# SciSharp/Gym.NET

Measured on AMD Instinct MI355X. Metric: env-steps/sec, higher is better.
Workload: dtype f32

## Files before the change

### gym.net_amd/csrc/lanes.hpp

```cpp
#pragma once
#include <hip/hip_runtime.h>
#include <stdint.h>

namespace gymnet {

template <class T, int N> struct VecOf { typedef T type __attribute__((ext_vector_type(N))); };
typedef float f32x4 __attribute__((ext_vector_type(4)));
typedef int32_t i32x4 __attribute__((ext_vector_type(4)));

template <class T, int VEC>
constexpr int piece_of() { return (int)(16 / sizeof(T)) < VEC ? (int)(16 / sizeof(T)) : VEC; }

template <class T, int VEC, bool NT, bool GUARD>
__device__ __forceinline__ void load_row(const T *__restrict__ p, int64_t i0, int64_t n, T (&v)[VEC]) {
    if constexpr (VEC > 1 && sizeof(T) > 1) {
        if (!GUARD || i0 + VEC <= n) {
            constexpr int P = piece_of<T, VEC>();
            static_assert(VEC % P == 0, "VEC must be a whole number of 16-byte pieces");
            typedef typename VecOf<T, P>::type V;
#pragma unroll
            for (int q = 0; q < VEC / P; ++q) {
                V t;
                if constexpr (NT) t = __builtin_nontemporal_load(reinterpret_cast<const V *>(p + i0 + q * P));
                else t = *reinterpret_cast<const V *>(p + i0 + q * P);
#pragma unroll
                for (int j = 0; j < P; ++j) v[q * P + j] = t[j];
            }
            return;
        }
    }
#pragma unroll
    for (int j = 0; j < VEC; ++j) {
        if (!GUARD || i0 + j < n) { if constexpr (NT) v[j] = __builtin_nontemporal_load(p + i0 + j); else v[j] = p[i0 + j]; }
        else v[j] = T(0);
    }
}

template <class T, int VEC, bool NT, bool GUARD>
__device__ __forceinline__ void store_row(T *__restrict__ p, int64_t i0, int64_t n, const T (&v)[VEC]) {
    if constexpr (VEC > 1 && sizeof(T) > 1) {
        if (!GUARD || i0 + VEC <= n) {
            constexpr int P = piece_of<T, VEC>();
            static_assert(P == 2 || P == 4, "16-byte pieces of 4- or 8-byte elements");
            typedef typename VecOf<T, P>::type V;
#pragma unroll
            for (int q = 0; q < VEC / P; ++q) {
                V t;
                if constexpr (P == 4) t = V{v[q * P], v[q * P + 1], v[q * P + 2], v[q * P + 3]};
                else t = V{v[q * P], v[q * P + 1]};
#ifdef GYMNET_PROBE_STORE_SC1
                if constexpr (NT && sizeof(T) == 4 && P == 4) {
                    asm volatile("global_store_dwordx4 %0, %1, off sc1" :: "v"(p + i0 + q * P), "v"(t) : "memory");
                    continue;
                }
#endif
                if constexpr (NT) __builtin_nontemporal_store(t, reinterpret_cast<V *>(p + i0 + q * P));
                else *reinterpret_cast<V *>(p + i0 + q * P) = t;
            }
            return;
        }
    }
#pragma unroll
    for (int j = 0; j < VEC; ++j)
        if (!GUARD || i0 + j < n) { if constexpr (NT) __builtin_nontemporal_store(v[j], p + i0 + j); else p[i0 + j] = v[j]; }
}

template <int VEC, bool NT, bool GUARD>
__device__ __forceinline__ void store_u8(uint8_t *__restrict__ p, int64_t i0, int64_t n, const uint8_t (&v)[VEC]) {
    if constexpr (VEC == 2) {
        if (!GUARD || i0 + 2 <= n) {
            const uint16_t w = (uint16_t)((uint16_t)v[0] | ((uint16_t)v[1] << 8));
            if constexpr (NT) __builtin_nontemporal_store(w, reinterpret_cast<uint16_t *>(p + i0));
            else *reinterpret_cast<uint16_t *>(p + i0) = w;
            return;
        }
    }
    if constexpr (VEC == 4) {
        if (!GUARD || i0 + 4 <= n) {
            const uint32_t w = (uint32_t)v[0] | ((uint32_t)v[1] << 8) | ((uint32_t)v[2] << 16) | ((uint32_t)v[3] << 24);
            if constexpr (NT) __builtin_nontemporal_store(w, reinterpret_cast<uint32_t *>(p + i0));
            else *reinterpret_cast<uint32_t *>(p + i0) = w;
            return;
        }
    }
#pragma unroll
    for (int j = 0; j < VEC; ++j)
        if (!GUARD || i0 + j < n) { if constexpr (NT) __builtin_nontemporal_store(v[j], p + i0 + j); else p[i0 + j] = v[j]; }
}

template <int VEC, bool NT, bool GUARD>
__device__ __forceinline__ void load_f32(const float *__restrict__ p, int64_t i0, int64_t n, float (&v)[VEC]) { load_row<float, VEC, NT, GUARD>(p, i0, n, v); }
template <int VEC, bool NT, bool GUARD>
__device__ __forceinline__ void store_f32(float *__restrict__ p, int64_t i0, int64_t n, const float (&v)[VEC]) { store_row<float, VEC, NT, GUARD>(p, i0, n, v); }
template <int VEC, bool NT, bool GUARD>
__device__ __forceinline__ void load_i32(const int32_t *__restrict__ p, int64_t i0, int64_t n, int32_t (&v)[VEC]) { load_row<int32_t, VEC, NT, GUARD>(p, i0, n, v); }
template <int VEC, bool NT, bool GUARD>
__device__ __forceinline__ void store_i32(int32_t *__restrict__ p, int64_t i0, int64_t n, const int32_t (&v)[VEC]) { store_row<int32_t, VEC, NT, GUARD>(p, i0, n, v); }

__device__ __forceinline__ uint32_t lane_id() {
    return __builtin_amdgcn_mbcnt_hi(~0u, __builtin_amdgcn_mbcnt_lo(~0u, 0u));
}

}
```

### gym.net_amd/csrc/step_kernels.hpp

```cpp
#pragma once
#include "kernels.hpp"

#include <cstdio>
#include <type_traits>

#include "lanes.hpp"
#include "philox.hpp"

namespace gymnet {

__device__ __forceinline__ float abs_real(float x) { return fabsf(x); }
__device__ __forceinline__ double abs_real(double x) { return __builtin_fabs(x); }

template <class Env, bool UNIFORM_KEY = false>
__device__ __forceinline__ void draw_reset(typename Env::Real (&s)[Env::S], uint64_t key, uint64_t lane, uint64_t tick) {
    if constexpr (Env::RESET_TAKES_KEY) Env::reset(s, key, lane, tick);
    else Env::reset(s, lane_words<UNIFORM_KEY>(key, lane, tick));
}

template <class Env>
__device__ __forceinline__ constexpr bool state_row_own(int k) {
    if constexpr (Env::OBS_ALIASES_STATE) return true; else return Env::OBS_ROW_OF_STATE[k] < 0;
}
template <class Env>
__device__ __forceinline__ const typename Env::Real *state_row_src(const typename Env::Real *state, int64_t state_stride,
                                                                    const typename Env::Real *obs_in, int64_t obs_stride, int k) {
    if constexpr (Env::OBS_ALIASES_STATE) return state + k * state_stride;
    else return Env::OBS_ROW_OF_STATE[k] < 0 ? state + k * state_stride : obs_in + Env::OBS_ROW_OF_STATE[k] * obs_stride;
}

__device__ __forceinline__ uint32_t wave_shard() {
    return (uint32_t)((((int64_t)blockIdx.x * blockDim.x + threadIdx.x) >> 6) & (kShards - 1));
}

template <int VEC, class Args>
__device__ __forceinline__ void count_after_done(const Args &a, const bool (&after)[VEC]) {
    uint32_t total = 0;
#pragma unroll
    for (int j = 0; j < VEC; ++j) total += (uint32_t)__popcll(__ballot(after[j]));
    if (total && lane_id() == (uint32_t)(__ffsll((unsigned long long)__ballot(1)) - 1))
        atomicAdd(&a.after_done[wave_shard() * kAfterStride], (unsigned long long)total);
}

template <class Env, bool AUTORESET, bool SMALL_ANGLE = false>
__device__ __forceinline__ void advance_sublane(typename Env::Real (&sj)[Env::S], typename Env::Action act, int32_t &sbd, float &rw,
                                                bool &dn, bool &after, bool in_range, typename Env::Real (&oj)[Env::O]) {
    if constexpr (Env::HAS_SMALL_ANGLE_PATH) Env::template step<SMALL_ANGLE, AUTORESET>(sj, act, rw, dn);
    else if constexpr (Env::OBS_ALIASES_STATE) Env::step(sj, act, rw, dn);
    else Env::step_observe(sj, act, rw, dn, oj);
    if constexpr (!AUTORESET && Env::HAS_SBD) {
        if (dn) {
            if (sbd == -1) { sbd = 0; }
            else { after = in_range; sbd += 1; rw = 0.0f; }
        }
    }
}

template <class Env, int VEC>
__device__ __forceinline__ bool wave_angles_small(const typename Env::Real (&s)[Env::S][VEC]) {
    if constexpr (!Env::HAS_SMALL_ANGLE_PATH) return false;
    else {
        bool small = true;
#pragma unroll
        for (int j = 0; j < VEC; ++j) small = small && (abs_real(s[Env::ANGLE_ROW][j]) <= Env::SMALL_ANGLE_BOUND);
        return __ballot(!small) == 0;
    }
}

template <class Env, int VEC, bool AUTORESET, bool GUARD, bool PACK = true>
__device__ __forceinline__ void advance_all(typename Env::Real (&s)[Env::S][VEC], typename Env::Action (&act)[VEC], int32_t (&sbd)[VEC],
                                            float (&rw)[VEC], bool (&dn)[VEC], bool (&after)[VEC], typename Env::Real (&o)[Env::O][VEC],
                                            int64_t i0, int64_t n) {
    constexpr int S = Env::S, O = Env::O;
    using Real = typename Env::Real;
#ifndef GYMNET_PROBE_NO_PACK
    constexpr bool kPack = true;
#else
    constexpr bool kPack = false;
#endif
    if constexpr (Env::PACKED2 && VEC == 2 && kPack && PACK) {
        Env::step_observe_x2(s, act, rw, dn, o);
    } else {
        auto all_sublanes = [&](auto small_tag) {
#pragma unroll
            for (int j = 0; j < VEC; ++j) {
// ... 85 lines not shown
    constexpr int S = Env::S;
    using Real = typename Env::Real;
    static_assert(Env::OBS_ALIASES_STATE, "the compacted reset hands back the state only");
    const uint32_t lane = lane_id();
    uint32_t rank[VEC];
    uint32_t total = 0;
#pragma unroll
    for (int j = 0; j < VEC; ++j) {
        const uint64_t m = __ballot((pending >> j) & 1u);
        rank[j] = total + __builtin_amdgcn_mbcnt_hi((uint32_t)(m >> 32), __builtin_amdgcn_mbcnt_lo((uint32_t)m, 0u));
        total += (uint32_t)__popcll(m);
    }
    if (total == 0) return;
    const int64_t wave_i0 = i0 - (int64_t)lane * VEC;
    constexpr bool SPLIT = has_split_reset<Env>();
    const uint32_t active = (uint32_t)__popcll(__ballot(1));
    const uint32_t A = SPLIT ? active >> 1 : active;
    if constexpr (SPLIT) {
        if (A == 0) {
            Real o_unused[Env::O][VEC];
            reset_pending<Env, VEC, LANE_SEEDS>(pending, s, o_unused, a, i0, n, tick);
            return;
        }
    }
    for (uint32_t base = 0; base < total; base += A) {
#pragma unroll
        for (int j = 0; j < VEC; ++j)
            if (((pending >> j) & 1u) && rank[j] - base < A) sc->slot[rank[j] - base] = lane * VEC + (uint32_t)j;
        wave_lds_fence();
        if constexpr (SPLIT) {
            const uint32_t r = lane >> 1, call = lane & 1u;
            const bool draws = r < A && r < total - base;
            PhiloxWords w{};
            if (kResetFullExec || draws) {
                const uint32_t sl = sc->slot[draws ? r : 0u];
                const int64_t gl = wave_i0 + (int64_t)sl;
                uint64_t key = a.seed;
                if constexpr (LANE_SEEDS) {
                    if (a.lane_seed && gl < n) key = a.lane_seed[gl];
                }
                w = lane_words(Env::reset_call_key(key, call), a.lane_offset + (uint64_t)gl, tick);
            }
            const PhiloxWords other = neighbour_words(w);
            if ((kResetFullExec || draws) && call == 0) {
                Real sj[S];
                Env::reset_from_words(sj, w, other);
#pragma unroll
                for (int k = 0; k < S; ++k) sc->draw[r][k] = sj[k];
            }
        } else if (kResetFullExec || lane < total - base) {
            const uint32_t sl = sc->slot[lane < total - base ? lane : 0u];
            const int64_t gl = wave_i0 + (int64_t)sl;
            Real sj[S];
            bool drawn = false;
            if constexpr (LANE_SEEDS) {
                if (a.lane_seed) {
                    draw_reset<Env, false>(sj, gl < n ? a.lane_seed[gl] : a.seed, a.lane_offset + (uint64_t)gl, tick);
                    drawn = true;
                }
            }
            if (!drawn) draw_reset<Env, true>(sj, a.seed, a.lane_offset + (uint64_t)gl, tick);
#pragma unroll
            for (int k = 0; k < S; ++k) sc->draw[lane][k] = sj[k];
        }
        wave_lds_fence();
        Real got[VEC][S];
#pragma unroll
        for (int j = 0; j < VEC; ++j) {
            const uint32_t r = rank[j] - base;
#pragma unroll
            for (int k = 0; k < S; ++k) got[j][k] = sc->draw[r < A ? r : 0u][k];
        }
#pragma unroll
        for (int j = 0; j < VEC; ++j) {
            const bool mine = ((pending >> j) & 1u) && rank[j] - base < A;
#pragma unroll
            for (int k = 0; k < S; ++k) s[k][j] = mine ? got[j][k] : s[k][j];
        }
        wave_lds_fence();
    }
}

template <int VEC>
__device__ __forceinline__ uint32_t rank_finished(const bool (&finished)[VEC], uint32_t (&off)[VEC]) {
    uint32_t total = 0;
#pragma unroll
    for (int j = 0; j < VEC; ++j) {
        const uint64_t m = __ballot(finished[j]);
        off[j] = total + __builtin_amdgcn_mbcnt_hi((uint32_t)(m >> 32), __builtin_amdgcn_mbcnt_lo((uint32_t)m, 0u));
        total += (uint32_t)__popcll(m);
    }
    return total;
}

template <class Env, int VEC>
__device__ __forceinline__ void append_done_records(const StepArgsT<typename Env::Real> &a, const bool (&finished)[VEC], int64_t i0,
                                                    const typename Env::Real (&s)[Env::S][VEC], const typename Env::Real (&o)[Env::O][VEC],
                                                    const float (&fin_ret)[VEC], const int32_t (&fin_len)[VEC], bool stats) {
    constexpr int S = Env::S, O = Env::O;
    const uint32_t lane = lane_id();
    uint32_t off[VEC];
    const uint32_t total = rank_finished<VEC>(finished, off);
    if (total) {
        const int leader = __ffsll((unsigned long long)__ballot(1)) - 1;
        const uint32_t shard = wave_shard();
        uint32_t base = 0;
        if ((int)lane == leader)
            base = atomicAdd(&a.done_count2[a.cparity * (kShards * kCountStride) + shard * kCountStride], total);
        base = __shfl(base, leader);
        const int64_t seg0 = (int64_t)shard * a.done_cap;
#pragma unroll
        for (int j = 0; j < VEC; ++j) {
            if (!finished[j]) continue;
            const int64_t pos = seg0 + base + off[j];
            a.done_list[pos] = (int32_t)(i0 + j);
            if (stats) { a.rec_ret[pos] = fin_ret[j]; a.rec_len[pos] = fin_len[j]; }
            if (a.rec_obs) {
#pragma unroll
                for (int k = 0; k < O; ++k)
                    a.rec_obs[((int64_t)shard * O + k) * a.done_cap + base + off[j]] = Env::OBS_ALIASES_STATE ? s[k < S ? k : 0][j] : o[k][j];
            }
        }
    }
}

template <class R>
__device__ __forceinline__ StepArgsT<R> hot_step_args(R *state, const void *action, int64_t n, int64_t state_stride, uint64_t *tick2, float *reward,
                                                      int32_t parity, const StepArgsT<R> &rest) {
    StepArgsT<R> a = rest;
    a.state = state; a.action = action; a.n = n; a.state_stride = state_stride; a.tick2 = tick2; a.reward = reward; a.parity = parity;
    return a;
}

template <class Env, int VEC>
struct LaneInputs {
    typename Env::Real s[Env::S][VEC];
    typename Env::Action act[VEC];
    int32_t sbd[VEC];
};

template <bool NT, class T>
__device__ __forceinline__ T load_elem(const T *p) { if constexpr (NT) return __builtin_nontemporal_load(p); else return *p; }

template <class T, int VEC, bool NT>
__device__ __forceinline__ void load_row_clamped(const T *__restrict__ p, int64_t i0, int64_t n, T (&v)[VEC]) {
#pragma unroll
    for (int j = 0; j < VEC; ++j) v[j] = load_elem<NT>(p + (i0 + j < n ? i0 + j : n - 1));
}

template <class Env, int VEC, bool AUTORESET, int NT>
__device__ __forceinline__ void load_inputs_clamped(const StepArgsT<typename Env::Real> &a, const int64_t i0, LaneInputs<Env, VEC> &in) {
    constexpr bool NT_SL = (NT & 1) != 0, NT_A = (NT & 4) != 0;
#pragma unroll
    for (int k = 0; k < Env::S; ++k)
        load_row_clamped<typename Env::Real, VEC, NT_SL>(state_row_src<Env>(a.state, a.state_stride, a.obs_in, a.obs_stride, k), i0, a.n, in.s[k]);
    if constexpr (Env::BOX_ACTION) load_row_clamped<float, VEC, NT_A>(static_cast<const float *>(a.action), i0, a.n, in.act);
    else load_row_clamped<int32_t, VEC, NT_A>(static_cast<const int32_t *>(a.action), i0, a.n, in.act);
#pragma unroll
    for (int j = 0; j < VEC; ++j) in.sbd[j] = 0;
    if constexpr (!AUTORESET && Env::HAS_SBD) load_row_clamped<int32_t, VEC, NT_SL>(a.sbd, i0, a.n, in.sbd);
}

template <class Env, int VEC, bool AUTORESET, int NT, bool GUARD>
__device__ __forceinline__ void load_inputs(const StepArgsT<typename Env::Real> &a, const int64_t i0, LaneInputs<Env, VEC> &in) {
    constexpr bool NT_SL = (NT & 1) != 0, NT_A = (NT & 4) != 0;
    if constexpr (GUARD) { load_inputs_clamped<Env, VEC, AUTORESET, NT>(a, i0, in); return; }
    const int64_t n = a.n;
#pragma unroll
    for (int k = 0; k < Env::S; ++k)
        load_row<typename Env::Real, VEC, NT_SL, GUARD>(state_row_src<Env>(a.state, a.state_stride, a.obs_in, a.obs_stride, k), i0, n, in.s[k]);
    if constexpr (Env::BOX_ACTION) load_f32<VEC, NT_A, GUARD>(static_cast<const float *>(a.action), i0, n, in.act);
    else load_i32<VEC, NT_A, GUARD>(static_cast<const int32_t *>(a.action), i0, n, in.act);
#pragma unroll
    for (int j = 0; j < VEC; ++j) in.sbd[j] = 0;
    if constexpr (!AUTORESET && Env::HAS_SBD) load_i32<VEC, NT_SL, GUARD>(a.sbd, i0, n, in.sbd);
}

template <class Env, int VEC, bool AUTORESET, bool EXTRAS, int NT, bool GUARD, int RESETF = 0, bool PACK = true>
__device__ __forceinline__ void advance_and_store(const StepArgsT<typename Env::Real> &a, const int64_t i0, const uint64_t tick,
                                                  LaneInputs<Env, VEC> &in, ResetScratch<Env> *sc = nullptr) {
    constexpr int S = Env::S, O = Env::O;
    using Real = typename Env::Real;
    constexpr bool NT_SS = (NT & 2) != 0, NT_O = (NT & 8) != 0;
    const int64_t n = a.n;
    Real (&s)[S][VEC] = in.s;
    typename Env::Action (&act)[VEC] = in.act;
    int32_t (&sbd)[VEC] = in.sbd;

    constexpr bool NT_SL = (NT & 1) != 0;
    float ep_ret[VEC], fin_ret[VEC];
    int32_t ep_len[VEC], fin_len[VEC];
    bool stats = false;
    if constexpr (EXTRAS) {
        stats = a.ep_ret != nullptr;
        if (stats) {
            if constexpr (GUARD) { load_row_clamped<float, VEC, NT_SL>(a.ep_ret, i0, n, ep_ret); load_row_clamped<int32_t, VEC, NT_SL>(a.ep_len, i0, n, ep_len); }
            else { load_f32<VEC, NT_SL, false>(a.ep_ret, i0, n, ep_ret); load_i32<VEC, NT_SL, false>(a.ep_len, i0, n, ep_len); }
        }
#pragma unroll
        for (int j = 0; j < VEC; ++j) { fin_ret[j] = 0.0f; fin_len[j] = 0; }
    }

    float reward[VEC];
    uint8_t done[VEC];
    bool finished[VEC];
    bool after[VEC];
#pragma unroll
    for (int j = 0; j < VEC; ++j) after[j] = false;
    Real o[O][VEC];
    uint32_t pending = 0;

    float rwv[VEC];
    bool dnv[VEC];
    advance_all<Env, VEC, AUTORESET, GUARD, PACK>(s, act, sbd, rwv, dnv, after, o, i0, n);

#pragma unroll
    for (int j = 0; j < VEC; ++j) {
        const float rw = rwv[j];
        uint8_t db = dnv[j] ? 1 : 0;
        if constexpr (EXTRAS) {
            if (stats) {
                ep_ret[j] += rw;
                ep_len[j] += 1;
                if (a.max_episode_steps > 0 && ep_len[j] >= a.max_episode_steps) db |= 2;
            }
        }
        const bool fin = db != 0;
        finished[j] = fin && (!GUARD || i0 + j < n);
        done[j] = db;
        reward[j] = rw;

        if constexpr (EXTRAS) {
            if (fin && a.final_obs && (!GUARD || i0 + j < n)) {
#pragma unroll
                for (int k = 0; k < O; ++k) a.final_obs[k * n + i0 + j] = Env::OBS_ALIASES_STATE ? s[k < S ? k : 0][j] : o[k][j];
            }
            if (stats && fin && (!GUARD || i0 + j < n)) {
                fin_ret[j] = ep_ret[j];
                fin_len[j] = ep_len[j];
                if (a.fin_ret) { a.fin_ret[i0 + j] = ep_ret[j]; a.fin_len[i0 + j] = ep_len[j]; }
                if constexpr (AUTORESET) { ep_ret[j] = 0.0f; ep_len[j] = 0; }
            }
        }

        if constexpr (AUTORESET) pending |= fin ? (1u << j) : 0u;
    }

    if constexpr (!AUTORESET && Env::HAS_SBD) count_after_done<VEC>(a, after);

    store_f32<VEC, NT_O, GUARD>(a.reward, i0, n, reward);
    store_u8<VEC, NT_O, GUARD>(a.done, i0, n, done);

    if constexpr (EXTRAS) {
        if (a.done_list) append_done_records<Env, VEC>(a, finished, i0, s, o, fin_ret, fin_len, stats);
    }

    if constexpr (AUTORESET && RESETF == 1) reset_pending_wave<Env, VEC, EXTRAS>(pending, s, a, i0, n, tick, sc);
    else if constexpr (AUTORESET) reset_pending<Env, VEC, EXTRAS>(pending, s, o, a, i0, n, tick);

#pragma unroll
    for (int k = 0; k < S; ++k)
        if (state_row_own<Env>(k)) store_row<Real, VEC, NT_SS, GUARD>(a.state_out + k * a.state_stride, i0, n, s[k]);
    if constexpr (!Env::OBS_ALIASES_STATE) {
#pragma unroll
        for (int k = 0; k < O; ++k) store_row<Real, VEC, NT_SS, GUARD>(a.obs + k * a.obs_stride, i0, n, o[k]);
    }
    if constexpr (!AUTORESET && Env::HAS_SBD) store_i32<VEC, NT_SS, GUARD>(a.sbd, i0, n, sbd);

    if constexpr (EXTRAS) {
        if (stats) { store_f32<VEC, NT_SS, GUARD>(a.ep_ret, i0, n, ep_ret); store_i32<VEC, NT_SS, GUARD>(a.ep_len, i0, n, ep_len); }
    }
}

template <class Env, int VEC, bool AUTORESET, bool EXTRAS, int NT, bool GUARD, int RESETF = 0>
__device__ __forceinline__ void step_body(const StepArgsT<typename Env::Real> &a, const int64_t i0, const uint64_t tick, ResetScratch<Env> *sc = nullptr) {
    LaneInputs<Env, VEC> in;
    load_inputs<Env, VEC, AUTORESET, NT, GUARD>(a, i0, in);
    advance_and_store<Env, VEC, AUTORESET, EXTRAS, NT, GUARD, RESETF>(a, i0, tick, in, sc);
}

template <class Env>
struct LaneOutputs { typename Env::Real s[Env::S], o[Env::O]; float reward; uint8_t done; int32_t sbd; };

template <class Env, bool AUTORESET>
__device__ __forceinline__ void compute_lane(const StepArgsT<typename Env::Real> &a, int64_t i, uint64_t tick, LaneInputs<Env, 1> &in,
                                             LaneOutputs<Env> &out) {
    constexpr int S = Env::S, O = Env::O;
    typename Env::Real o[O][1];
    float rw[1];
    bool dn[1], after[1] = {false};
    advance_all<Env, 1, AUTORESET, false>(in.s, in.act, in.sbd, rw, dn, after, o, i, a.n);
    if constexpr (!AUTORESET && Env::HAS_SBD) count_after_done<1>(a, after);
    if constexpr (AUTORESET) reset_pending<Env, 1, false>(dn[0] ? 1u : 0u, in.s, o, a, i, a.n, tick);
#pragma unroll
    for (int k = 0; k < S; ++k) out.s[k] = in.s[k][0];
#pragma unroll
    for (int k = 0; k < O; ++k) out.o[k] = o[k][0];
    out.reward = rw[0]; out.done = dn[0] ? 1 : 0; out.sbd = in.sbd[0];
}

template <class Env, bool AUTORESET, int NT>
__device__ __forceinline__ void store_lane(const StepArgsT<typename Env::Real> &a, int64_t i, const LaneOutputs<Env> &out) {
    constexpr bool NT_SS = (NT & 2) != 0, NT_O = (NT & 8) != 0;
    auto st = [](auto *p, auto v, bool nt) { if (nt) __builtin_nontemporal_store(v, p); else *p = v; };
    st(a.reward + i, out.reward, NT_O);
    if constexpr (NT_O) __builtin_nontemporal_store(out.done, a.done + i); else a.done[i] = out.done;
#pragma unroll
    for (int k = 0; k < Env::S; ++k)
        if (state_row_own<Env>(k)) st(a.state_out + k * a.state_stride + i, out.s[k], NT_SS);
    if constexpr (!Env::OBS_ALIASES_STATE) {
#pragma unroll
        for (int k = 0; k < Env::O; ++k) st(a.obs + k * a.obs_stride + i, out.o[k], NT_SS);
    }
    if constexpr (!AUTORESET && Env::HAS_SBD) a.sbd[i] = out.sbd;
}

template <class Env, int ITEMS, bool AUTORESET, int NT>
__global__ __launch_bounds__(256) void step_kernel_pipe(typename Env::Real *state, const void *action, int64_t n, int64_t state_stride, uint64_t *tick2,
                                                        float *reward, int32_t block, int32_t parity, const StepArgsT<typename Env::Real> rest) {
    const StepArgsT<typename Env::Real> a = hot_step_args(state, action, n, state_stride, tick2, reward, parity, rest);
    const uint64_t tick = a.tick2[a.parity];
    if (blockIdx.x == 0 && threadIdx.x == 0) a.tick2[a.parity ^ 1] = tick + 1;
    const int64_t T = (int64_t)gridDim.x * block;
    const int64_t i = (int64_t)blockIdx.x * block + threadIdx.x;
    LaneInputs<Env, 1> in[ITEMS];
#pragma unroll
    for (int k = 0; k < ITEMS; ++k) {
        const int64_t idx = i + k * T;
        load_inputs<Env, 1, AUTORESET, NT, false>(a, idx < a.n ? idx : a.n - 1, in[k]);
    }
#pragma unroll
    for (int k = 0; k < ITEMS; ++k) {
        LaneOutputs<Env> out;
        if (k == 0) {
#pragma unroll
            for (int c = 0; c < Env::S; ++c) asm volatile("" : "+v"(in[0].s[c][0]));
            asm volatile("" : "+v"(in[0].act[0]));
        }
        compute_lane<Env, AUTORESET>(a, i + k * T, tick, in[k], out);
        if (k == 0) {
#pragma unroll
            for (int kk = 1; kk < ITEMS; ++kk) {
#pragma unroll
                for (int c = 0; c < Env::S; ++c) asm volatile("" : "+v"(in[kk].s[c][0]), "+v"(out.s[Env::S - 1]));
                asm volatile("" : "+v"(in[kk].act[0]), "+v"(out.reward));
            }
        }
        if (i + k * T < a.n) store_lane<Env, AUTORESET, NT>(a, i + k * T, out);
    }
}

template <class Env>
struct DeferScratch {
    uint32_t slot[32];
    typename Env::Real draw[32][Env::S];
};

template <class Env, int PAIRS, class StateOf>
__device__ __forceinline__ void reset_group_deferred(uint32_t pending, StateOf s, const StepArgsT<typename Env::Real> &a, int64_t t_wave0,
                                                     int64_t T, int first_pair, uint64_t tick, DeferScratch<Env> *sc) {
    static_assert(Env::RESET_CALLS == 2 && 2 * PAIRS <= 8, "two lanes per reset; the slot word keeps 3 bits for the sub-lane position");
// ... 142 lines not shown
constexpr int own_state_rows() { int c = 0; for (int k = 0; k < Env::S; ++k) c += state_row_own<Env>(k) ? 1 : 0; return c; }

template <class Env, int TPB, bool AUTORESET, int NT, int CW = 8>
__global__ __launch_bounds__(CW * 64 + 64) void step_kernel_lds(const StepArgs a, const int64_t tiles) {
    static_assert(std::is_same<typename Env::Real, float>::value, "the producer / consumer form stages float rows through LDS");
    constexpr int kLdsComputeWaves = CW, kLdsTile = CW * 64;
    constexpr int S = Env::S, O = Env::O;
    constexpr int NOWN = own_state_rows<Env>();
    constexpr int NROW = NOWN + (Env::OBS_ALIASES_STATE ? 0 : O) + 1;
    constexpr bool NT_SS = (NT & 2) != 0, NT_O = (NT & 8) != 0;
    __shared__ float out_buf[2][NROW][kLdsTile];
    __shared__ uint8_t done_buf[2][kLdsTile];
    const uint64_t tick = a.tick2[a.parity];
    if (blockIdx.x == 0 && threadIdx.x == 0) a.tick2[a.parity ^ 1] = tick + 1;
    const int lane = threadIdx.x & 63;
    const bool storer = (threadIdx.x >> 6) == kLdsComputeWaves;
    const int cl = threadIdx.x;
    const int64_t t0 = (int64_t)blockIdx.x * TPB;
    const int nt = (int)(tiles - t0 < TPB ? tiles - t0 : TPB);

    auto tile_barrier = [] { asm volatile("s_waitcnt lgkmcnt(0)\n\ts_barrier" ::: "memory"); };

    LaneInputs<Env, 1> in[TPB + 1];
    if (!storer) load_inputs<Env, 1, AUTORESET, NT, false>(a, t0 * kLdsTile + cl, in[0]);
#pragma unroll
    for (int s = 0; s <= TPB; ++s) {
        if (!storer) {
            if (s < TPB) {
                const int64_t i = (t0 + (s < nt ? s : nt - 1)) * kLdsTile + cl;
                const int64_t ip = (t0 + (s + 1 < nt ? s + 1 : nt - 1)) * kLdsTile + cl;
                load_inputs<Env, 1, AUTORESET, NT, false>(a, ip, in[s + 1]);
#pragma unroll
                for (int c = 0; c < S; ++c) asm volatile("" : "+v"(in[s].s[c][0]));
                asm volatile("" : "+v"(in[s].act[0]));
                LaneOutputs<Env> out;
                compute_lane<Env, AUTORESET>(a, i, tick, in[s], out);
#pragma unroll
                for (int c = 0; c < S; ++c) asm volatile("" : "+v"(in[s + 1].s[c][0]), "+v"(out.s[S - 1]));
                asm volatile("" : "+v"(in[s + 1].act[0]), "+v"(out.reward));
                if (s < nt) {
                    int r = 0;
#pragma unroll
                    for (int k = 0; k < S; ++k)
                        if (state_row_own<Env>(k)) out_buf[s & 1][r++][cl] = out.s[k];
                    if constexpr (!Env::OBS_ALIASES_STATE) {
#pragma unroll
                        for (int k = 0; k < O; ++k) out_buf[s & 1][r++][cl] = out.o[k];
                    }
                    out_buf[s & 1][r][cl] = out.reward;
                    done_buf[s & 1][cl] = out.done;
                }
            }
        } else if (s >= 1 && s - 1 < nt) {
            const int b = (s - 1) & 1;
            const int64_t base = (t0 + s - 1) * kLdsTile;
            auto drain = [&](float *row, int r, bool nt_store) {
#pragma unroll
                for (int j = 0; j < kLdsTile / 256; ++j) {
                    const f32x4 v = *reinterpret_cast<const f32x4 *>(&out_buf[b][r][j * 256 + lane * 4]);
                    f32x4 *dst = reinterpret_cast<f32x4 *>(row + base + j * 256 + lane * 4);
                    if (nt_store) __builtin_nontemporal_store(v, dst); else *dst = v;
                }
                static_assert(kLdsTile % 256 == 0, "the storing wave moves 256 floats per instruction");
            };
            int r = 0;
#pragma unroll
            for (int k = 0; k < S; ++k)
                if (state_row_own<Env>(k)) drain(a.state_out + k * a.state_stride, r++, NT_SS);
            if constexpr (!Env::OBS_ALIASES_STATE) {
#pragma unroll
                for (int k = 0; k < O; ++k) drain(a.obs + k * a.obs_stride, r++, NT_SS);
            }
            drain(a.reward, r, NT_O);
            if (lane < kLdsTile / 16) {
                const i32x4 v = *reinterpret_cast<const i32x4 *>(&done_buf[b][lane * 16]);
                i32x4 *dst = reinterpret_cast<i32x4 *>(a.done + base + lane * 16);
                if constexpr (NT_O) __builtin_nontemporal_store(v, dst); else *dst = v;
            }
        }
        tile_barrier();
    }
}

template <class Env, int VEC, bool AUTORESET, bool EXTRAS, int NT, int RESETF = 0>
__global__ __launch_bounds__(256) void step_kernel(typename Env::Real *state, const void *action, int64_t n, int64_t state_stride, uint64_t *tick2,
                                                   float *reward, int32_t block, int32_t parity, const StepArgsT<typename Env::Real> rest) {
    const StepArgsT<typename Env::Real> a = hot_step_args(state, action, n, state_stride, tick2, reward, parity, rest);
    const int64_t i0 = ((int64_t)blockIdx.x * block + threadIdx.x) * VEC;
    ResetScratch<Env> *sc = nullptr;
    if constexpr (RESETF == 1) {
        __shared__ ResetScratch<Env> scratch[256 / 64];
        sc = &scratch[threadIdx.x >> 6];
    }
    const uint64_t tick = a.tick2[a.parity];
    if (blockIdx.x == 0 && threadIdx.x == 0) {
        a.tick2[a.parity ^ 1] = tick + 1;
    }
    if constexpr (EXTRAS) {
        if (blockIdx.x == 0 && a.done_count2)
            for (int sh = threadIdx.x; sh < kShards; sh += block) a.done_count2[(a.cparity ^ 1) * (kShards * kCountStride) + sh * kCountStride] = 0u;
    }
    if (((int64_t)blockIdx.x + 1) * block * VEC <= a.n) {
        step_body<Env, VEC, AUTORESET, EXTRAS, NT, false, RESETF>(a, i0, tick, sc);
    } else {
        if (i0 >= a.n) return;
        step_body<Env, VEC, AUTORESET, EXTRAS, NT, true, RESETF>(a, i0, tick, sc);
    }
}

template <class Env>
__device__ __forceinline__ typename Env::Action sampled_action(uint32_t word_a) {
    if constexpr (Env::BOX_ACTION) return Env::ACTION_LOW + (Env::ACTION_HIGH - Env::ACTION_LOW) * u01_24(word_a);
    else return (int32_t)__umulhi(word_a, (uint32_t)Env::ACTION_N);
}

template <int VEC>
__device__ __forceinline__ void thread_action_words(uint64_t seed, uint64_t gl0, uint64_t tick, bool want_aux, bool one_group,
                                                    uint32_t (&wa)[VEC], uint32_t (&wb)[VEC]) {
    static_assert(VEC == 1 || VEC == 2 || VEC == 4, "a thread's lanes must fit one group of four");
    if (one_group) {
        const PhiloxWords r = action_group_words<true>(seed, gl0 >> 2, tick);
        PhiloxWords c{};
        if (want_aux) c = aux_group_words<true>(seed, gl0 >> 2, tick);
        const uint32_t base = (uint32_t)gl0 & 3u;
        if constexpr (VEC == 4) {
#pragma unroll
            for (int j = 0; j < 4; ++j) { wa[j] = r.w[j]; wb[j] = c.w[j]; }
        } else if constexpr (VEC == 2) {
#pragma unroll
            for (int j = 0; j < 2; ++j) { wa[j] = base ? r.w[2 + j] : r.w[j]; wb[j] = base ? c.w[2 + j] : c.w[j]; }
        } else {
            wa[0] = word_of(r, base); wb[0] = word_of(c, base);
        }
    } else {
#pragma unroll
        for (int j = 0; j < VEC; ++j) { wa[j] = 0u; wb[j] = 0u; }
#pragma unroll 1
        for (int j = 0; j < VEC; ++j) {
            const uint32_t a = action_word<true>(seed, gl0 + (uint64_t)j, tick);
            const uint32_t b = want_aux ? aux_word<true>(seed, gl0 + (uint64_t)j, tick) : 0u;
#pragma unroll
            for (int k = 0; k < VEC; ++k) { wa[k] = k == j ? a : wa[k]; wb[k] = k == j ? b : wb[k]; }
        }
    }
}

constexpr uint32_t kStageRecords = 256;
struct EpisodeStage { int32_t t[kStageRecords], lane[kStageRecords]; float ret[kStageRecords]; int32_t len[kStageRecords]; };

template <class Env, int VEC, bool AUTORESET, bool GUARD, bool EXTRAS, bool SAMPLE, int RESETF = 0, int RECORDS = 0>
__device__ __forceinline__ void rollout_body(const StepArgsT<typename Env::Real> &a, const RolloutArgsT<typename Env::Real> &ro,
                                             const int64_t i0, const uint64_t tick0, ResetScratch<Env> *sc = nullptr, EpisodeStage *stage = nullptr) {
    constexpr int S = Env::S, O = Env::O;
    using Act = typename Env::Action;
    using Real = typename Env::Real;
    const int64_t n = a.n;

    Real s[S][VEC];
#pragma unroll
    for (int k = 0; k < S; ++k) load_row<Real, VEC, true, GUARD>(state_row_src<Env>(a.state, a.state_stride, a.obs_in, a.obs_stride, k), i0, n, s[k]);
    int32_t sbd[VEC] = {};
    if constexpr (!AUTORESET && Env::HAS_SBD) load_i32<VEC, true, GUARD>(a.sbd, i0, n, sbd);

    auto load_action = [&](int64_t slice, Act (&dst)[VEC]) {
        const char *base = static_cast<const char *>(a.action) + (size_t)(slice * ro.action_stride) * 4;
        if constexpr (Env::BOX_ACTION) load_f32<VEC, true, GUARD>(reinterpret_cast<const float *>(base), i0, n, dst);
        else load_i32<VEC, true, GUARD>(reinterpret_cast<const int32_t *>(base), i0, n, dst);
    };

    Act act[VEC], act_next[VEC];
    bool use_ring = true;
    const bool one_group = (a.lane_offset % (uint64_t)VEC) == 0;
    const uint32_t explore_at_or_below = coin_threshold(ro.epsilon);
    if constexpr (SAMPLE) {
        use_ring = ro.action_source == 2;
#pragma unroll
        for (int j = 0; j < VEC; ++j) { act[j] = Act(0); act_next[j] = Act(0); }
        if (use_ring) load_action(0, act);
    } else {
        load_action(0, act);
    }
    int64_t slice = 0;
    float reward[VEC];
    uint8_t done[VEC];
    Real o[O][VEC];

    float ep_ret[VEC], fin_ret[VEC];
    int32_t ep_len[VEC], fin_len[VEC];
    bool stats = false;
    if constexpr (EXTRAS) {
// ... 540 lines not shown
```

Measured before the change: 159.4 billion.

## Split lane addressing into scalar base plus 32-bit offset and trim step kernel head

Adds a LaneSplit position type that keeps the workgroup base in scalar registers and uses a 32-bit per-thread offset, so the unguarded full-tile path can use cheaper address arithmetic and issue its loads before the tick read and bookkeeping. It reads the tick through the constant address space, tests the tail with a scalar high-word check, and adds a sched_barrier after the first state row load. It also adds an optional compacted reset path driven by ballot masks (DIET), which is disabled by default. The gain depends on the kernel head being a meaningful share of a short memory-bound kernel; the inline-asm tricks could hurt scheduling.

```diff
diff --git a/gym.net_amd/csrc/lanes.hpp b/gym.net_amd/csrc/lanes.hpp
--- a/gym.net_amd/csrc/lanes.hpp
+++ b/gym.net_amd/csrc/lanes.hpp
@@ -1,6 +1,7 @@
 #pragma once
 #include <hip/hip_runtime.h>
 #include <stdint.h>
+#include <type_traits>
 
 namespace gymnet {
 
@@ -101,4 +102,42 @@
     return __builtin_amdgcn_mbcnt_hi(~0u, __builtin_amdgcn_mbcnt_lo(~0u, 0u));
 }
 
+struct LaneIndex {
+    int64_t i0;
+    __device__ __forceinline__ int64_t lane() const { return i0; }
+    __device__ __forceinline__ int64_t wave_first(int vec) const { return i0 - (int64_t)lane_id() * vec; }
+    template <class T> __device__ __forceinline__ T *at(T *row) const { return row + i0; }
+};
+struct LaneSplit {
+    uint64_t wg0;
+    uint32_t t;
+    __device__ __forceinline__ int64_t lane() const { return (int64_t)(wg0 + t); }
+    __device__ __forceinline__ int64_t wave_first(int vec) const {
+        return (int64_t)(wg0 + (uint32_t)__builtin_amdgcn_readfirstlane((int)(t - lane_id() * (uint32_t)vec)));
+    }
+    template <class T> __device__ __forceinline__ T *at(T *row) const {
+        typedef typename std::conditional<std::is_const<T>::value, const char, char>::type Byte;
+        typedef __attribute__((address_space(1))) Byte GlobalByte;
+        uint64_t base = reinterpret_cast<uint64_t>(row) + wg0 * sizeof(T);
+        asm("" : "+s"(base));
+        return reinterpret_cast<T *>((Byte *)(reinterpret_cast<GlobalByte *>(base) + (uint32_t)(t * (uint32_t)sizeof(T))));
+    }
+};
+
+template <class T, int VEC, bool NT, bool GUARD, class Pos>
+__device__ __forceinline__ void load_row_at(const T *__restrict__ p, const Pos &pos, int64_t n, T (&v)[VEC]) {
+    if constexpr (GUARD) load_row<T, VEC, NT, true>(p, pos.lane(), n, v);
+    else load_row<T, VEC, NT, false>(pos.at(p), 0, n, v);
 }
+template <class T, int VEC, bool NT, bool GUARD, class Pos>
+__device__ __forceinline__ void store_row_at(T *__restrict__ p, const Pos &pos, int64_t n, const T (&v)[VEC]) {
+    if constexpr (GUARD) store_row<T, VEC, NT, true>(p, pos.lane(), n, v);
+    else store_row<T, VEC, NT, false>(pos.at(p), 0, n, v);
+}
+template <int VEC, bool NT, bool GUARD, class Pos>
+__device__ __forceinline__ void store_u8_at(uint8_t *__restrict__ p, const Pos &pos, int64_t n, const uint8_t (&v)[VEC]) {
+    if constexpr (GUARD) store_u8<VEC, NT, true>(p, pos.lane(), n, v);
+    else store_u8<VEC, NT, false>(pos.at(p), 0, n, v);
+}
+
+}
diff --git a/gym.net_amd/csrc/step_kernels.hpp b/gym.net_amd/csrc/step_kernels.hpp
--- a/gym.net_amd/csrc/step_kernels.hpp
+++ b/gym.net_amd/csrc/step_kernels.hpp
@@ -1,6 +1,7 @@
 #pragma once
 #include "kernels.hpp"
 
+#include <cstddef>
 #include <cstdio>
 #include <type_traits>
 
@@ -252,6 +253,128 @@
 }
 
 template <int VEC>
+__device__ __forceinline__ uint32_t rank_masks(const uint64_t (&mask)[VEC], uint32_t (&off)[VEC]) {
+    uint32_t total = 0;
+#pragma unroll
+    for (int j = 0; j < VEC; ++j) {
+        off[j] = total + __builtin_amdgcn_mbcnt_hi((uint32_t)(mask[j] >> 32), __builtin_amdgcn_mbcnt_lo((uint32_t)mask[j], 0u));
+        total += (uint32_t)__popcll(mask[j]);
+    }
+    return total;
+}
+
+template <class Env, int VEC, bool LANE_SEEDS, bool ONE>
+__device__ __forceinline__ void reset_finished_round(const uint32_t base, const uint32_t total, const uint32_t A, const uint32_t lane,
+                                                     const uint32_t (&rank)[VEC], const bool (&fin_flag)[VEC], const uint64_t (&mask)[VEC],
+                                                     typename Env::Real (&s)[Env::S][VEC],
+                                                     const StepArgsT<typename Env::Real> &a, int64_t wave_i0, int64_t n, uint64_t tick,
+                                                     ResetScratch<Env> *sc) {
+    constexpr int S = Env::S;
+    using Real = typename Env::Real;
+    constexpr bool SPLIT = has_split_reset<Env>();
+    bool fin[VEC];
+#pragma unroll
+    for (int j = 0; j < VEC; ++j) fin[j] = ONE ? __builtin_amdgcn_inverse_ballot_w64(mask[j]) : fin_flag[j];
+    {
+        if constexpr (ONE) {
+            static_assert(offsetof(ResetScratch<Env>, draw) == 64 * sizeof(uint32_t) && sizeof(sc->draw) >= 64 * sizeof(uint32_t), "park word");
+            uint32_t *const words = reinterpret_cast<uint32_t *>(sc);
+            const uint32_t park = 64u + lane;
+#pragma unroll
+            for (int j = 0; j < VEC; ++j) words[fin[j] ? rank[j] : park] = lane * VEC + (uint32_t)j;
+        } else {
+#pragma unroll
+            for (int j = 0; j < VEC; ++j)
+                if (fin[j] && rank[j] - base < A) sc->slot[rank[j] - base] = lane * VEC + (uint32_t)j;
+        }
+        wave_lds_fence();
+        if constexpr (SPLIT) {
+            const uint32_t r = lane >> 1, call = lane & 1u;
+            const bool draws = r < A && r < total - base;
+            PhiloxWords w{};
+            if (kResetFullExec || draws) {
+                const uint32_t sl = sc->slot[draws ? r : 0u];
+                const int64_t gl = wave_i0 + (int64_t)sl;
+                uint64_t key = a.seed;
+                if constexpr (LANE_SEEDS) {
+                    if (a.lane_seed && gl < n) key = a.lane_seed[gl];
+                }
+                w = lane_words(Env::reset_call_key(key, call), a.lane_offset + (uint64_t)gl, tick);
+            }
+            const PhiloxWords other = neighbour_words(w);
+            if ((kResetFullExec || draws) && call == 0) {
+                Real sj[S];
+                Env::reset_from_words(sj, w, other);
+#pragma unroll
+                for (int k = 0; k < S; ++k) sc->draw[r][k] = sj[k];
+            }
+        } else if (kResetFullExec || lane < total - base) {
+            const uint32_t sl = sc->slot[lane < total - base ? lane : 0u];
+            const int64_t gl = wave_i0 + (int64_t)sl;
+            Real sj[S];
+            bool drawn = false;
+            if constexpr (LANE_SEEDS) {
+                if (a.lane_seed) {
+                    draw_reset<Env, false>(sj, gl < n ? a.lane_seed[gl] : a.seed, a.lane_offset + (uint64_t)gl, tick);
+                    drawn = true;
+                }
+            }
+            if (!drawn) draw_reset<Env, true>(sj, a.seed, a.lane_offset + (uint64_t)gl, tick);
+#pragma unroll
+            for (int k = 0; k < S; ++k) sc->draw[lane][k] = sj[k];
+        }
+        wave_lds_fence();
+        Real got[VEC][S];
+#pragma unroll
+        for (int j = 0; j < VEC; ++j) {
+            const uint32_t r = rank[j] - base;
+            const uint32_t row = ONE ? (r & 63u) : (r < A ? r : 0u);
+#pragma unroll
+            for (int k = 0; k < S; ++k) got[j][k] = sc->draw[row][k];
+        }
+#pragma unroll
+        for (int j = 0; j < VEC; ++j) {
+            const bool mine = ONE ? fin[j] : (fin[j] && rank[j] - base < A);
+#pragma unroll
+            for (int k = 0; k < S; ++k) s[k][j] = mine ? got[j][k] : s[k][j];
+        }
+        wave_lds_fence();
+    }
+}
+
+template <class Env, int VEC, bool LANE_SEEDS>
+__device__ __forceinline__ void reset_finished_wave(const bool (&fin)[VEC], const uint64_t (&mask)[VEC], typename Env::Real (&s)[Env::S][VEC],
+                                                    const StepArgsT<typename Env::Real> &a, int64_t i0, int64_t wave_i0, int64_t n, uint64_t tick,
+                                                    ResetScratch<Env> *sc) {
+    constexpr int S = Env::S;
+    using Real = typename Env::Real;
+    static_assert(Env::OBS_ALIASES_STATE, "the compacted reset hands back the state only");
+    uint32_t rank[VEC];
+    const uint32_t total = rank_masks<VEC>(mask, rank);
+    if (total == 0) return;
+    const uint32_t lane = lane_id();
+    constexpr bool SPLIT = has_split_reset<Env>();
+    const uint32_t active = (uint32_t)__popcll(__ballot(1));
+    const uint32_t A = SPLIT ? active >> 1 : active;
+    if constexpr (SPLIT) {
+        if (A == 0) {
+            uint32_t pending = 0;
+#pragma unroll
+            for (int j = 0; j < VEC; ++j) pending |= fin[j] ? (1u << j) : 0u;
+            Real o_unused[Env::O][VEC];
+            reset_pending<Env, VEC, LANE_SEEDS>(pending, s, o_unused, a, i0, n, tick);
+            return;
+        }
+    }
+    if (total <= A) {
+        reset_finished_round<Env, VEC, LANE_SEEDS, true>(0u, total, A, lane, rank, fin, mask, s, a, wave_i0, n, tick, sc);
+    } else {
+        for (uint32_t base = 0; base < total; base += A)
+            reset_finished_round<Env, VEC, LANE_SEEDS, false>(base, total, A, lane, rank, fin, mask, s, a, wave_i0, n, tick, sc);
+    }
+}
+
+template <int VEC>
 __device__ __forceinline__ uint32_t rank_finished(const bool (&finished)[VEC], uint32_t (&off)[VEC]) {
     uint32_t total = 0;
 #pragma unroll
@@ -264,13 +387,12 @@
 }
 
 template <class Env, int VEC>
-__device__ __forceinline__ void append_done_records(const StepArgsT<typename Env::Real> &a, const bool (&finished)[VEC], int64_t i0,
-                                                    const typename Env::Real (&s)[Env::S][VEC], const typename Env::Real (&o)[Env::O][VEC],
-                                                    const float (&fin_ret)[VEC], const int32_t (&fin_len)[VEC], bool stats) {
+__device__ __forceinline__ void append_ranked_records(const StepArgsT<typename Env::Real> &a, const bool (&finished)[VEC], const uint32_t (&off)[VEC],
+                                                      const uint32_t total, int64_t i0, const typename Env::Real (&s)[Env::S][VEC],
+                                                      const typename Env::Real (&o)[Env::O][VEC], const float (&fin_ret)[VEC],
+                                                      const int32_t (&fin_len)[VEC], bool stats) {
     constexpr int S = Env::S, O = Env::O;
     const uint32_t lane = lane_id();
-    uint32_t off[VEC];
-    const uint32_t total = rank_finished<VEC>(finished, off);
     if (total) {
         const int leader = __ffsll((unsigned long long)__ballot(1)) - 1;
         const uint32_t shard = wave_shard();
@@ -294,6 +416,15 @@
     }
 }
 
+template <class Env, int VEC>
+__device__ __forceinline__ void append_done_records(const StepArgsT<typename Env::Real> &a, const bool (&finished)[VEC], int64_t i0,
+                                                    const typename Env::Real (&s)[Env::S][VEC], const typename Env::Real (&o)[Env::O][VEC],
+                                                    const float (&fin_ret)[VEC], const int32_t (&fin_len)[VEC], bool stats) {
+    uint32_t off[VEC];
+    const uint32_t total = rank_finished<VEC>(finished, off);
+    append_ranked_records<Env, VEC>(a, finished, off, total, i0, s, o, fin_ret, fin_len, stats);
+}
+
 template <class R>
 __device__ __forceinline__ StepArgsT<R> hot_step_args(R *state, const void *action, int64_t n, int64_t state_stride, uint64_t *tick2, float *reward,
                                                       int32_t parity, const StepArgsT<R> &rest) {
@@ -331,28 +462,35 @@
     if constexpr (!AUTORESET && Env::HAS_SBD) load_row_clamped<int32_t, VEC, NT_SL>(a.sbd, i0, a.n, in.sbd);
 }
 
+template <class Env, int VEC, bool AUTORESET, int NT, bool GUARD, class Pos>
+__device__ __forceinline__ void load_inputs(const StepArgsT<typename Env::Real> &a, const Pos &pos, LaneInputs<Env, VEC> &in) {
+    constexpr bool NT_SL = (NT & 1) != 0, NT_A = (NT & 4) != 0;
+    if constexpr (GUARD) { load_inputs_clamped<Env, VEC, AUTORESET, NT>(a, pos.lane(), in); return; }
+    const int64_t n = a.n;
+#pragma unroll
+    for (int k = 0; k < Env::S; ++k) {
+        load_row_at<typename Env::Real, VEC, NT_SL, GUARD>(state_row_src<Env>(a.state, a.state_stride, a.obs_in, a.obs_stride, k), pos, n, in.s[k]);
+        if constexpr (std::is_same<Pos, LaneSplit>::value) { if (k == 0) __builtin_amdgcn_sched_barrier(0); }
+    }
+    if constexpr (Env::BOX_ACTION) load_row_at<float, VEC, NT_A, GUARD>(static_cast<const float *>(a.action), pos, n, in.act);
+    else load_row_at<int32_t, VEC, NT_A, GUARD>(static_cast<const int32_t *>(a.action), pos, n, in.act);
+#pragma unroll
+    for (int j = 0; j < VEC; ++j) in.sbd[j] = 0;
+    if constexpr (!AUTORESET && Env::HAS_SBD) load_row_at<int32_t, VEC, NT_SL, GUARD>(a.sbd, pos, n, in.sbd);
+}
 template <class Env, int VEC, bool AUTORESET, int NT, bool GUARD>
 __device__ __forceinline__ void load_inputs(const StepArgsT<typename Env::Real> &a, const int64_t i0, LaneInputs<Env, VEC> &in) {
-    constexpr bool NT_SL = (NT & 1) != 0, NT_A = (NT & 4) != 0;
-    if constexpr (GUARD) { load_inputs_clamped<Env, VEC, AUTORESET, NT>(a, i0, in); return; }
-    const int64_t n = a.n;
-#pragma unroll
-    for (int k = 0; k < Env::S; ++k)
-        load_row<typename Env::Real, VEC, NT_SL, GUARD>(state_row_src<Env>(a.state, a.state_stride, a.obs_in, a.obs_stride, k), i0, n, in.s[k]);
-    if constexpr (Env::BOX_ACTION) load_f32<VEC, NT_A, GUARD>(static_cast<const float *>(a.action), i0, n, in.act);
-    else load_i32<VEC, NT_A, GUARD>(static_cast<const int32_t *>(a.action), i0, n, in.act);
-#pragma unroll
-    for (int j = 0; j < VEC; ++j) in.sbd[j] = 0;
-    if constexpr (!AUTORESET && Env::HAS_SBD) load_i32<VEC, NT_SL, GUARD>(a.sbd, i0, n, in.sbd);
-}
-
-template <class Env, int VEC, bool AUTORESET, bool EXTRAS, int NT, bool GUARD, int RESETF = 0, bool PACK = true>
-__device__ __forceinline__ void advance_and_store(const StepArgsT<typename Env::Real> &a, const int64_t i0, const uint64_t tick,
+    load_inputs<Env, VEC, AUTORESET, NT, GUARD>(a, LaneIndex{i0}, in);
+}
+
+template <class Env, int VEC, bool AUTORESET, bool EXTRAS, int NT, bool GUARD, int RESETF = 0, bool PACK = true, bool DIET = false, class Pos>
+__device__ __forceinline__ void advance_and_store(const StepArgsT<typename Env::Real> &a, const Pos &pos, const uint64_t tick,
                                                   LaneInputs<Env, VEC> &in, ResetScratch<Env> *sc = nullptr) {
     constexpr int S = Env::S, O = Env::O;
     using Real = typename Env::Real;
     constexpr bool NT_SS = (NT & 2) != 0, NT_O = (NT & 8) != 0;
     const int64_t n = a.n;
+    const int64_t i0 = pos.lane();
     Real (&s)[S][VEC] = in.s;
     typename Env::Action (&act)[VEC] = in.act;
     int32_t (&sbd)[VEC] = in.sbd;
@@ -365,7 +503,7 @@
         stats = a.ep_ret != nullptr;
         if (stats) {
             if constexpr (GUARD) { load_row_clamped<float, VEC, NT_SL>(a.ep_ret, i0, n, ep_ret); load_row_clamped<int32_t, VEC, NT_SL>(a.ep_len, i0, n, ep_len); }
-            else { load_f32<VEC, NT_SL, false>(a.ep_ret, i0, n, ep_ret); load_i32<VEC, NT_SL, false>(a.ep_len, i0, n, ep_len); }
+            else { load_row_at<float, VEC, NT_SL, false>(a.ep_ret, pos, n, ep_ret); load_row_at<int32_t, VEC, NT_SL, false>(a.ep_len, pos, n, ep_len); }
         }
 #pragma unroll
         for (int j = 0; j < VEC; ++j) { fin_ret[j] = 0.0f; fin_len[j] = 0; }
@@ -418,35 +556,57 @@
 
     if constexpr (!AUTORESET && Env::HAS_SBD) count_after_done<VEC>(a, after);
 
-    store_f32<VEC, NT_O, GUARD>(a.reward, i0, n, reward);
-    store_u8<VEC, NT_O, GUARD>(a.done, i0, n, done);
+    store_row_at<float, VEC, NT_O, GUARD>(a.reward, pos, n, reward);
+    store_u8_at<VEC, NT_O, GUARD>(a.done, pos, n, done);
+
+    constexpr bool kDietReset = DIET && AUTORESET && RESETF == 1;
+    uint64_t fin_mask[VEC];
+    if constexpr (DIET && (EXTRAS || kDietReset)) {
+#pragma unroll
+        for (int j = 0; j < VEC; ++j) fin_mask[j] = __ballot(finished[j]);
+    }
 
     if constexpr (EXTRAS) {
-        if (a.done_list) append_done_records<Env, VEC>(a, finished, i0, s, o, fin_ret, fin_len, stats);
-    }
-
-    if constexpr (AUTORESET && RESETF == 1) reset_pending_wave<Env, VEC, EXTRAS>(pending, s, a, i0, n, tick, sc);
+        if (a.done_list) {
+            if constexpr (DIET) {
+                uint32_t off[VEC];
+                const uint32_t total = rank_masks<VEC>(fin_mask, off);
+                append_ranked_records<Env, VEC>(a, finished, off, total, i0, s, o, fin_ret, fin_len, stats);
+            } else {
+                append_done_records<Env, VEC>(a, finished, i0, s, o, fin_ret, fin_len, stats);
+            }
+        }
+    }
+
+    if constexpr (kDietReset) reset_finished_wave<Env, VEC, EXTRAS>(finished, fin_mask, s, a, i0, pos.wave_first(VEC), n, tick, sc);
+    else if constexpr (AUTORESET && RESETF == 1) reset_pending_wave<Env, VEC, EXTRAS>(pending, s, a, i0, n, tick, sc);
     else if constexpr (AUTORESET) reset_pending<Env, VEC, EXTRAS>(pending, s, o, a, i0, n, tick);
 
 #pragma unroll
     for (int k = 0; k < S; ++k)
-        if (state_row_own<Env>(k)) store_row<Real, VEC, NT_SS, GUARD>(a.state_out + k * a.state_stride, i0, n, s[k]);
+        if (state_row_own<Env>(k)) store_row_at<Real, VEC, NT_SS, GUARD>(a.state_out + k * a.state_stride, pos, n, s[k]);
     if constexpr (!Env::OBS_ALIASES_STATE) {
 #pragma unroll
-        for (int k = 0; k < O; ++k) store_row<Real, VEC, NT_SS, GUARD>(a.obs + k * a.obs_stride, i0, n, o[k]);
-    }
-    if constexpr (!AUTORESET && Env::HAS_SBD) store_i32<VEC, NT_SS, GUARD>(a.sbd, i0, n, sbd);
+        for (int k = 0; k < O; ++k) store_row_at<Real, VEC, NT_SS, GUARD>(a.obs + k * a.obs_stride, pos, n, o[k]);
+    }
+    if constexpr (!AUTORESET && Env::HAS_SBD) store_row_at<int32_t, VEC, NT_SS, GUARD>(a.sbd, pos, n, sbd);
 
     if constexpr (EXTRAS) {
-        if (stats) { store_f32<VEC, NT_SS, GUARD>(a.ep_ret, i0, n, ep_ret); store_i32<VEC, NT_SS, GUARD>(a.ep_len, i0, n, ep_len); }
-    }
-}
-
-template <class Env, int VEC, bool AUTORESET, bool EXTRAS, int NT, bool GUARD, int RESETF = 0>
+        if (stats) { store_row_at<float, VEC, NT_SS, GUARD>(a.ep_ret, pos, n, ep_ret); store_row_at<int32_t, VEC, NT_SS, GUARD>(a.ep_len, pos, n, ep_len); }
+    }
+}
+
+template <class Env, int VEC, bool AUTORESET, bool EXTRAS, int NT, bool GUARD, int RESETF = 0, bool PACK = true>
+__device__ __forceinline__ void advance_and_store(const StepArgsT<typename Env::Real> &a, const int64_t i0, const uint64_t tick,
+                                                  LaneInputs<Env, VEC> &in, ResetScratch<Env> *sc = nullptr) {
+    advance_and_store<Env, VEC, AUTORESET, EXTRAS, NT, GUARD, RESETF, PACK, false>(a, LaneIndex{i0}, tick, in, sc);
+}
+
+template <class Env, int VEC, bool AUTORESET, bool EXTRAS, int NT, bool GUARD, int RESETF = 0, bool DIET = false>
 __device__ __forceinline__ void step_body(const StepArgsT<typename Env::Real> &a, const int64_t i0, const uint64_t tick, ResetScratch<Env> *sc = nullptr) {
     LaneInputs<Env, VEC> in;
     load_inputs<Env, VEC, AUTORESET, NT, GUARD>(a, i0, in);
-    advance_and_store<Env, VEC, AUTORESET, EXTRAS, NT, GUARD, RESETF>(a, i0, tick, in, sc);
+    advance_and_store<Env, VEC, AUTORESET, EXTRAS, NT, GUARD, RESETF, true, DIET>(a, LaneIndex{i0}, tick, in, sc);
 }
 
 template <class Env>
@@ -755,30 +915,78 @@
     }
 }
 
+template <class Env, int VEC, bool AUTORESET, bool EXTRAS, int NT, int RESETF, bool HEAD, bool DIET>
+__device__ __forceinline__ void step_kernel_body(typename Env::Real *state, const void *action, int64_t n, int64_t state_stride, uint64_t *tick2,
+                                                 float *reward, int32_t block, int32_t parity, const StepArgsT<typename Env::Real> &rest) {
+    const StepArgsT<typename Env::Real> a = hot_step_args(state, action, n, state_stride, tick2, reward, parity, rest);
+    auto wave_scratch = [&](const uint32_t wave) -> ResetScratch<Env> * {
+        if constexpr (RESETF == 1) {
+            __shared__ ResetScratch<Env> scratch[256 / 64];
+            return &scratch[wave];
+        } else {
+            return nullptr;
+        }
+    };
+    auto read_tick = [&]() -> uint64_t {
+        typedef const __attribute__((address_space(4))) uint64_t ConstTick;
+        if constexpr (HEAD) return ((ConstTick *)a.tick2)[(uint32_t)a.parity & 1u];
+        else return a.tick2[a.parity];
+    };
+    auto for_next_launch = [&](const uint64_t tick) {
+        if constexpr (HEAD) {
+            if (blockIdx.x != 0) return;
+            if (threadIdx.x == 0) a.tick2[((uint32_t)a.parity & 1u) ^ 1u] = tick + 1;
+        } else if (blockIdx.x == 0 && threadIdx.x == 0) {
+            a.tick2[a.parity ^ 1] = tick + 1;
+        }
+        if constexpr (EXTRAS) {
+            if (blockIdx.x == 0 && a.done_count2)
+                for (int sh = threadIdx.x; sh < kShards; sh += block) a.done_count2[(a.cparity ^ 1) * (kShards * kCountStride) + sh * kCountStride] = 0u;
+        }
+    };
+    if constexpr (!HEAD) {
+        ResetScratch<Env> *const sc = wave_scratch(threadIdx.x >> 6);
+        const uint64_t tick = read_tick();
+        const int64_t i0 = ((int64_t)blockIdx.x * block + threadIdx.x) * VEC;
+        for_next_launch(tick);
+        if (((int64_t)blockIdx.x + 1) * block * VEC <= a.n) {
+            step_body<Env, VEC, AUTORESET, EXTRAS, NT, false, RESETF, DIET>(a, i0, tick, sc);
+        } else {
+            if (i0 >= a.n) return;
+            step_body<Env, VEC, AUTORESET, EXTRAS, NT, true, RESETF, DIET>(a, i0, tick, sc);
+        }
+    } else {
+        const uint32_t wg_lanes = (uint32_t)block * VEC;
+        const uint64_t wg0 = (uint64_t)blockIdx.x * wg_lanes;
+        int32_t slack_hi = (int32_t)((uint64_t)(a.n - (int64_t)(wg0 + wg_lanes)) >> 32);
+        asm volatile("" : "+s"(slack_hi));
+        if (__builtin_expect(slack_hi < 0, 0)) {
+            ResetScratch<Env> *const sc = wave_scratch(threadIdx.x >> 6);
+            const uint64_t tick = read_tick();
+            for_next_launch(tick);
+            const int64_t i0 = (int64_t)(wg0 + (uint32_t)threadIdx.x * VEC);
+            if (i0 >= a.n) return;
+            step_body<Env, VEC, AUTORESET, EXTRAS, NT, true, RESETF, DIET>(a, i0, tick, sc);
+        } else {
+            const LaneSplit pos{wg0, (uint32_t)threadIdx.x * VEC};
+            LaneInputs<Env, VEC> in;
+            load_inputs<Env, VEC, AUTORESET, NT, false>(a, pos, in);
+            uint32_t wave = threadIdx.x >> 6;
+            asm volatile("" : "+v"(wave));
+            ResetScratch<Env> *const sc = wave_scratch(wave & 3u);
+            const uint64_t tick = read_tick();
+            for_next_launch(tick);
+            advance_and_store<Env, VEC, AUTORESET, EXTRAS, NT, false, RESETF, true, DIET>(a, pos, tick, in, sc);
+        }
+    }
+}
+
+constexpr bool kHotHead = true, kHotDiet = false;
+
 template <class Env, int VEC, bool AUTORESET, bool EXTRAS, int NT, int RESETF = 0>
 __global__ __launch_bounds__(256) void step_kernel(typename Env::Real *state, const void *action, int64_t n, int64_t state_stride, uint64_t *tick2,
                                                    float *reward, int32_t block, int32_t parity, const StepArgsT<typename Env::Real> rest) {
-    const StepArgsT<typename Env::Real> a = hot_step_args(state, action, n, state_stride, tick2, reward, parity, rest);
-    const int64_t i0 = ((int64_t)blockIdx.x * block + threadIdx.x) * VEC;
-    ResetScratch<Env> *sc = nullptr;
-    if constexpr (RESETF == 1) {
-        __shared__ ResetScratch<Env> scratch[256 / 64];
-        sc = &scratch[threadIdx.x >> 6];
-    }
-    const uint64_t tick = a.tick2[a.parity];
-    if (blockIdx.x == 0 && threadIdx.x == 0) {
-        a.tick2[a.parity ^ 1] = tick + 1;
-    }
-    if constexpr (EXTRAS) {
-        if (blockIdx.x == 0 && a.done_count2)
-            for (int sh = threadIdx.x; sh < kShards; sh += block) a.done_count2[(a.cparity ^ 1) * (kShards * kCountStride) + sh * kCountStride] = 0u;
-    }
-    if (((int64_t)blockIdx.x + 1) * block * VEC <= a.n) {
-        step_body<Env, VEC, AUTORESET, EXTRAS, NT, false, RESETF>(a, i0, tick, sc);
-    } else {
-        if (i0 >= a.n) return;
-        step_body<Env, VEC, AUTORESET, EXTRAS, NT, true, RESETF>(a, i0, tick, sc);
-    }
+    step_kernel_body<Env, VEC, AUTORESET, EXTRAS, NT, RESETF, kHotHead, kHotDiet>(state, action, n, state_stride, tick2, reward, block, parity, rest);
 }
 
 template <class Env>
```

Result: no change. 158.7 billion, median of 2 (-0.5%).
